# gnovack/distributed-training-and-deepspeed

Measured on AMD Instinct MI355X. Metric: tokens/sec (whole node) BERT-base DDP, higher is better.
Workload: dtype bf16; 1 GPU; model=bert-base-cased, params=108340804, global_batch=1024, per_gpu_batch=1024, seq_len=512, parallelism=dp1, grad_dtype=bfloat16, impl=fused, mlm_head=sparse (labelled rows only, static capacity 80896; identical loss/grads), optimizer=fused AdamW (transformers.AdamW hyper-params, lr 5e-5), tuned_gemms=True, hip_graph=False, force_collectives=False, prewarm=auto, async_wgrad=False, opt_overlap=True

## Files before the change

### distributed_training_and_deepspeed_amd/ops/_lib.py

```python
from __future__ import annotations

import ctypes
import os
from pathlib import Path
import threading

import torch

from . import build as _build

_LIB = None
_LOCK = threading.Lock()

P = ctypes.c_void_p
I = ctypes.c_int
F = ctypes.c_float
SZ = ctypes.c_size_t
U32 = ctypes.c_uint32
L = ctypes.c_long

_SIGS = {
    "dtd_ln_bwd_num_partials": (I, [I, I]),
    "dtd_ln_fwd": (I, [I, P, P, P, P, P, P, P, P, I, I, F, F, P, U32, P]),
    "dtd_ln_bwd": (I, [I, P, P, P, P, P, P, P, P, P, P, P, P, I, I, F, P, U32, P]),
# ... 28 lines not shown
    "dtd_embed_fwd": (I, [I, P, P, P, P, P, P, I, I, I, I, P]),
    "dtd_embed_fwd_pos": (I, [I, P, P, P, P, P, P, P, I, I, I, I, P]),
    "dtd_embed_word_bwd": (I, [I, I, P, P, P, P, I, I, I, I, P]),
    "dtd_embed_pos_bwd": (I, [I, I, P, P, I, I, I, I, I, P]),
    "dtd_scatter_rows": (I, [P, P, P, I, P, I, I, P]),
    "dtd_dropout": (I, [I, P, P, P, SZ, F, P, U32, P]),
    "dtd_embed_ln_fwd": (I, [P, P, P, P, P, P, P, P, P, P, P, I, I, I, I, F, F, P, U32, P]),
    "dtd_adam_step": (I, [P, P, P, P, I, P, SZ, P, I, P]),
    "dtd_scale_cast": (I, [P, I, P, I, SZ, F, P, P]),
    "dtd_sqnorm_num_partials": (I, [SZ]),
    "dtd_sqnorm_partials": (I, [P, I, SZ, P, P]),
    "dtd_attn_fwd": (I, [P, P, P, P, P, P, P, I, I, I, I, I, I, I, F, F, P, U32, P]),
    "dtd_attn_bwd": (I, [P, P, P, P, P, P, P, P, P, P, P, P, I, I, I, I, I, I, I, F, F, P, P]),
    "dtd_attn_fwd_range": (I, [P, P, P, P, P, P, P, I, I, I, I, I, I, I, F, F, P, U32, P, P]),
    "dtd_attn_bwd_range": (I, [P, P, P, P, P, P, P, P, P, P, P, P, I, I, I, I, I, I, I, F, F, P, P, P]),
    "dtd_attn_fwd_doc": (I, [P, P, P, P, P, P, P, I, I, I, I, I, I, I, F, F, P, U32, P, P]),
    "dtd_attn_bwd_doc": (I, [P, P, P, P, P, P, P, P, P, P, P, P, I, I, I, I, I, I, I, F, F, P, P, P]),
    "dtd_attn_fwd_gqa": (I, [P, P, P, P, P, I, I, I, I, I, I, I, I, F, P, P, P]),
    "dtd_attn_bwd_gqa": (I, [P, P, P, P, P, P, P, P, P, P, I, I, I, I, I, I, I, I, F, P, P, P]),
    "dtd_attn_masks": (I, [P, I, I, I, F, P, U32, P]),
    "dtd_attn_set_bwd_form": (I, [I]),
    "dtd_attn_set_bwd_kernels": (I, [I]),
    "dtd_attn_fused_bwd_built": (I, []),
    "dtd_attn_fwd_f32": (I, [P, P, P, P, P, P, P, I, I, I, I, I, I, I, F, F, P]),
    "dtd_attn_bwd_f32": (I, [P, P, P, P, P, P, P, P, P, P, P, P, I, I, I, I, I, I, I, F, F, P]),
    "dtd_softmax_fwd": (I, [I, P, P, I, I, P]),
    "dtd_softmax_bwd": (I, [I, P, P, P, I, I, P]),
    "dtd_gemm_bt_supported": (I, [I, I, I]),
    "dtd_gemm_w4_supported": (I, [I, I, I]),
    "dtd_gemm_w4_set_sched": (I, [I]),
    "dtd_gemm_w4": (I, [I, P, I, P, I, P, I, P, I, I, I, P]),
    "dtd_gemm_bt_part_rows": (I, [I]),
    "dtd_gemm_bt": (I, [I, P, I, P, I, P, I, P, P, I, P, P, I, I, I, P, P]),
    "dtd_spin_occupy": (I, [I, ctypes.c_double, P]),
    "dtd_gemm_set_stagger": (I, [ctypes.c_double]),
    "dtd_transpose_bf16": (I, [P, P, I, I, P]),
    "dtd_transpose_many": (I, [P, P, P, P, I, P]),
    "dtd_gemm_set_stamps": (I, [P]),
    "dtd_wgrad_tn_supported": (I, [I, I, I]),
    "dtd_wgrad_tn_splits": (I, [I, I, I]),
    "dtd_wgrad_tn": (I, [I, P, I, P, I, P, I, I, I, I, P]),
    "dtd_gemm_f32_supported": (I, [I, I, I]),
    "dtd_gemm_f32_set_kernel": (I, [I]),
    "dtd_gemm_f32_nt": (I, [P, I, P, I, P, I, P, I, I, I, I, P]),
    "dtd_gemm_f32_nn": (I, [P, I, P, I, P, I, I, I, I, I, P]),
    "dtd_transpose_many_f32": (I, [P, P, P, P, I, P]),
    "dtd_gemm_f32_tn_splits": (I, [I, I, I]),
    "dtd_gemm_f32_tn": (I, [P, I, P, I, P, I, I, I, I, P]),
    "dtd_gemm_ln_supported": (I, [I, I, I, I, I, I, I]),
    "dtd_gemm_ln": (I, [P, P, P, P, P, P, P, P, P, P, I, I, I, I, I, I, I, F, F, P, U32, P]),
    "dtd_splitk_reduce": (I, [P, I, I, ctypes.c_longlong, P, I, I, P]),
}


class KernelError(RuntimeError):
    pass


def available() -> bool:
    return torch.cuda.is_available()


def lib():
    global _LIB
    if _LIB is not None:
        return _LIB
# ... 58 lines not shown
```

### distributed_training_and_deepspeed_amd/ops/csrc/gemm.hip

```cpp
#include <type_traits>

#ifndef DTD_GEMM_DIAG
#define DTD_GEMM_DIAG 0
#endif
#ifndef DTD_GEMM_ONEBAR
#define DTD_GEMM_ONEBAR 0
#endif
constexpr bool kOneBar = DTD_GEMM_ONEBAR != 0;

#include "common.h"

using namespace dtd;

namespace {

typedef __attribute__((address_space(3))) void lds_void;
typedef const __attribute__((address_space(1))) void gbl_void;

constexpr int BM = 256, BN = 256, BK = 64;
constexpr int A_BYTES = BM * BK * 2;
constexpr int TILE_BYTES = (BM + BN) * BK * 2;
constexpr int LDS_BYTES = 2 * TILE_BYTES;

enum Epi : int { EPI_STORE = 0, EPI_BIAS_GELU = 1, EPI_GELU_BWD = 2, EPI_ADD = 3, EPI_BIAS_GELU_TANH = 4,
                 EPI_GELU_TANH_BWD = 5, EPI_BIAS_RELU = 6, EPI_RELU_BWD = 7, EPI_BIAS_GELU_G = 8,
                 EPI_BIAS_GELU_TANH_G = 9, EPI_MUL_BWD = 10, EPI_LAST = EPI_MUL_BWD };
__host__ __device__ constexpr bool is_gelu_fwd(int e) {
  return e == EPI_BIAS_GELU || e == EPI_BIAS_GELU_TANH || e == EPI_BIAS_RELU || e == EPI_BIAS_GELU_G ||
         e == EPI_BIAS_GELU_TANH_G;
}
__host__ __device__ constexpr bool is_gelu_bwd(int e) {
  return e == EPI_GELU_BWD || e == EPI_GELU_TANH_BWD || e == EPI_RELU_BWD || e == EPI_MUL_BWD;
}
__host__ __device__ constexpr bool stores_grad(int e) { return e == EPI_BIAS_GELU_G || e == EPI_BIAS_GELU_TANH_G; }

struct GemmArgs {
  const bf16* a; const bf16* b;
  bf16* c;
  bf16* c2;
  const bf16* u;
  const bf16* bias;
  float* part;
  int M, N, K, lda, ldb, ldc, ldu;
  unsigned long long* stamps;
  int* sched;
  int stagger;
  int nt;
};

__device__ __forceinline__ void st8(bf16* p, const bf16x8& v, int nt) {
  if (nt) __builtin_nontemporal_store(v, reinterpret_cast<bf16x8*>(p));
  else *reinterpret_cast<bf16x8*>(p) = v;
}

constexpr int SCHED_DONE = 8;

#ifdef DTD_GEMM_STAMPS
#define STAMP(slot, iter)                                                                          \
  do {                                                                                             \
    if (g.stamps && tid == 0 && (iter) < 32)                                                       \
      g.stamps[((size_t)blockIdx.x * 32 + (iter)) * 8 + (slot)] = __builtin_amdgcn_s_memtime();    \
  } while (0)
#define STAMP_ID(iter)                                                                             \
  do {                                                                                             \
    if (g.stamps && tid == 0 && (iter) < 32)                                                       \
      g.stamps[((size_t)blockIdx.x * 32 + (iter)) * 8 + 7] =                                       \
          ((unsigned long long)__builtin_amdgcn_s_getreg((31 << 11) | 20) << 32) |                 \
          __builtin_amdgcn_s_getreg((31 << 11) | 4);                                               \
  } while (0)
#else
#define STAMP(slot, iter) do {} while (0)
#define STAMP_ID(iter) do {} while (0)
#endif

__device__ __forceinline__ void bar() {
  asm volatile("" ::: "memory");
  __builtin_amdgcn_s_barrier();
  asm volatile("" ::: "memory");
}

// ... 33 lines not shown
__device__ __forceinline__ float epi_act_grad(float x) {
  if constexpr (EPI == EPI_GELU_TANH_BWD) return gelu_tanh_grad(x);
  else if constexpr (EPI == EPI_RELU_BWD) return x > 0.f ? 1.f : 0.f;
  else if constexpr (EPI == EPI_MUL_BWD) return x;
  else return gelu_grad(x);
}
template <int EPI>
__device__ __forceinline__ void epi_act_and_grad(float x, float& a, float& d) {
  if constexpr (EPI == EPI_BIAS_GELU_TANH_G) {
    const float k = 0.7978845608028654f;
    const float t = tanh_fast(k * fmaf(0.044715f * x, x * x, x));
    const float h = 0.5f * (1.f + t);
    a = x * h;
    d = h + 0.5f * x * (1.f - t * t) * k * (1.f + 3.f * 0.044715f * x * x);
  } else {
    const float e = gauss_e(x);
    const float cdf = phi_cdf(x, e);
    a = x * cdf;
    d = fmaf(x * 0.3989422804014327f, e, cdf);
  }
}
__device__ __forceinline__ float gelu_grad(float x) {
  const float e = gauss_e(x);
  return fmaf(x * 0.3989422804014327f, e, phi_cdf(x, e));
}

__device__ __forceinline__ bf16x4 cvt4(f32x4 v) {
  typedef float f32x2_t __attribute__((ext_vector_type(2)));
  const bf16x2 lo = __builtin_convertvector(f32x2_t{v[0], v[1]}, bf16x2);
  const bf16x2 hi = __builtin_convertvector(f32x2_t{v[2], v[3]}, bf16x2);
  return __builtin_shufflevector(lo, hi, 0, 1, 2, 3);
}

template <int EPI>
__device__ __forceinline__ void act_and_grad8(const bf16x8& v, float (&a)[8], float (&d)[8]) {
  float x[8];
#pragma unroll
  for (int j = 0; j < 8; ++j) x[j] = (float)v[j];
  if constexpr (EPI == EPI_BIAS_GELU_TANH_G) {
#pragma unroll
    for (int j = 0; j < 8; ++j) epi_act_and_grad<EPI>(x[j], a[j], d[j]);
  } else {
    float e[8], t[8], p[8], c[8];
#pragma unroll
    for (int j = 0; j < 8; ++j) e[j] = gauss_e(x[j]);
#pragma unroll
    for (int j = 0; j < 8; ++j) t[j] = __builtin_amdgcn_rcpf(fmaf(fabsf(x[j]), 0.3275911f * 0.70710678118654752f, 1.f));
#pragma unroll
    for (int j = 0; j < 8; ++j) p[j] = fmaf(t[j], 1.061405429f, -1.453152027f);
#pragma unroll
    for (int j = 0; j < 8; ++j) p[j] = fmaf(t[j], p[j], 1.421413741f);
#pragma unroll
    for (int j = 0; j < 8; ++j) p[j] = fmaf(t[j], p[j], -0.284496736f);
#pragma unroll
    for (int j = 0; j < 8; ++j) p[j] = t[j] * fmaf(t[j], p[j], 0.254829592f);
#pragma unroll
    for (int j = 0; j < 8; ++j) c[j] = 0.5f + 0.5f * copysignf(1.f - p[j] * e[j], x[j]);
#pragma unroll
    for (int j = 0; j < 8; ++j) {
      a[j] = x[j] * c[j];
      d[j] = fmaf(x[j] * 0.3989422804014327f, e[j], c[j]);
    }
  }
}
__device__ __forceinline__ bf16x8 cvt8(const float (&f)[8]) {
  const bf16x4 lo = cvt4(f32x4{f[0], f[1], f[2], f[3]}), hi = cvt4(f32x4{f[4], f[5], f[6], f[7]});
  return __builtin_shufflevector(lo, hi, 0, 1, 2, 3, 4, 5, 6, 7);
}

__device__ __forceinline__ int xcd_remap(int id, int n) {
  const int q = n / 8, r = n % 8, x = id % 8;
  return (x < r ? x * (q + 1) : r * (q + 1) + (x - r) * q) + id / 8;
}

__device__ __forceinline__ __amdgpu_buffer_rsrc_t uniform_rsrc(const void* p) {
  const uint64_t a = (uint64_t)p;
  const uint32_t lo = __builtin_amdgcn_readfirstlane((uint32_t)a);
  const uint32_t hi = __builtin_amdgcn_readfirstlane((uint32_t)(a >> 32));
  return __builtin_amdgcn_make_buffer_rsrc((void*)(((uint64_t)hi << 32) | lo), (short)0, 0x7fffffff, 0x00020000);
}

struct StageOffs {
  int a[2][2], b[2][2];
  int la[2][2], lb[2][2];
};

__device__ __forceinline__ StageOffs stage_offsets(int w, int lane, int lda, int ldb) {
  StageOffs o;
  const int dr = lane >> 3;
  const int sc = ((lane & 7) ^ dr) * 8;
#pragma unroll
  for (int h = 0; h < 2; ++h)
#pragma unroll
    for (int i = 0; i < 2; ++i) {
      const int j = w * 2 + i;
      const int ra = (j >> 3) * 128 + (h ? 64 : 0) + 8 * (j & 7);
      const int rb = (j >> 2) * 64 + (h ? 32 : 0) + 8 * (j & 3);
      o.a[h][i] = ((ra + dr) * lda + sc) * 2;
      o.b[h][i] = ((rb + dr) * ldb + sc) * 2;
      o.la[h][i] = ra * 128;
// ... 201 lines not shown
    __syncthreads();
    float* red = reinterpret_cast<float*>(smem);
    if (lane < 32) {
      *reinterpret_cast<f32x4*>(red + w * 256 + c * 8) = f32x4{colsum[0], colsum[1], colsum[2], colsum[3]};
      *reinterpret_cast<f32x4*>(red + w * 256 + c * 8 + 4) = f32x4{colsum[4], colsum[5], colsum[6], colsum[7]};
    }
    __syncthreads();
    if (tid < 256) {
      float s = 0.f;
#pragma unroll
      for (int k = 0; k < 8; ++k) s += red[k * 256 + tid];
      g.part[(size_t)bm * g.N + n0 + tid] = s;
    }
  }
}

constexpr int kStores(int epi) {
  return is_gelu_fwd(epi) ? 32 : is_gelu_bwd(epi) ? 32 : epi == EPI_ADD ? 48 : 16;
}

__device__ __forceinline__ void tile_of(int t, int ntn, int& m0, int& n0) {
  m0 = (t / ntn) * BM;
  n0 = (t % ntn) * BN;
}

__device__ __forceinline__ void sched_finish(int* q, int nwg, int tid) {
  if (q == nullptr || tid != 0) return;
  if (atomicAdd(&q[SCHED_DONE], 1) == nwg - 1) {
#pragma unroll
    for (int i = 0; i <= SCHED_DONE; ++i) atomicExch(&q[i], 0);
  }
}

template <int EPI, bool DYN>
__global__ void __launch_bounds__(512, 2) gemm_bt_persistent(GemmArgs g) {
  __shared__ __attribute__((aligned(1024))) char smem[LDS_BYTES];
  const int tid = threadIdx.x, lane = tid & 63, w = __builtin_amdgcn_readfirstlane(tid >> 6);
  const int li = lane & 15, lq = lane >> 4, sw = li & 7;
  const int wm = w >> 2, wn = w & 3;
  const int ntn = g.N / BN, ntiles = (g.M / BM) * ntn;
  const int nk = g.K / BK;
  const int nwg = gridDim.x, x = blockIdx.x % 8, l = blockIdx.x / 8, per = nwg / 8;
  const int q = ntiles / 8, r = ntiles % 8;
  const int beg = x < r ? x * (q + 1) : r * (q + 1) + (x - r) * q;
  const int end = beg + q + (x < r ? 1 : 0);
  constexpr bool dyn = DYN;
  __shared__ int qslot[2];
  int t = beg + l;
  if (t >= end) {
    if constexpr (DYN) sched_finish(g.sched, nwg, tid);
    return;
  }
  if (g.stagger > 0 && (l & 1)) {
    const unsigned long long t0 = __builtin_amdgcn_s_memrealtime();
    while (__builtin_amdgcn_s_memrealtime() - t0 < (unsigned long long)g.stagger) __builtin_amdgcn_s_sleep(8);
  }
  int m0, n0;
  tile_of(t, ntn, m0, n0);
  const StageOffs so = stage_offsets(w, lane, g.lda, g.ldb);
  auto rsa = uniform_rsrc(g.a + (size_t)m0 * g.lda), rsb = uniform_rsrc(g.b + (size_t)n0 * g.ldb);
  stage<0>(so, rsa, rsb, smem, 0);
  stage<1>(so, rsa, rsb, smem, 0);
  stage<2>(so, rsa, rsb, smem, 0);
  stage<3>(so, rsa, rsb, smem, 0);
  asm volatile("s_waitcnt vmcnt(0)" ::: "memory");
  __syncthreads();
  if (!kOneBar && __builtin_amdgcn_readfirstlane(wm) == 1) bar();

  const int arow = (wm * 128 + li) * 128;
  const int brow = A_BYTES + (wn * 64 + li) * 128;
  const int ch0 = ((0 * 4 + lq) ^ sw) * 16, ch1 = ((1 * 4 + lq) ^ sw) * 16;
  constexpr int S = kStores(EPI);
  constexpr int WAIT_FIRST = 4 + S > 63 ? 63 : 4 + S;

  bf16x8 af[4][2], b0[2][2], b1[2][2];
  f32x4 acc[8][4];
  int buf = 0;
  int it = 0;
  STAMP_ID(0);
  while (true) {
    STAMP(0, it);
    const int tn = dyn && it > 0 ? __builtin_amdgcn_readfirstlane(qslot[it & 1]) : t + per;
    const bool has_next = tn < end;
    int m1 = 0, n1 = 0;
    if (has_next) tile_of(tn, ntn, m1, n1);
    const auto rsa1 = uniform_rsrc(g.a + (size_t)m1 * g.lda), rsb1 = uniform_rsrc(g.b + (size_t)n1 * g.ldb);
    auto kstep = [&](auto first_c, int kt) {
      constexpr bool first = decltype(first_c)::value;
      const char* cur = smem + buf * TILE_BYTES;
      char* nxt = smem + (buf ^ 1) * TILE_BYTES;
      buf ^= 1;
      const bool more_here = kt + 1 < nk;
      const bool more = more_here || has_next;
// ... 113 lines not shown
    bar();
    char* img = smem + (buf ^ 1) * TILE_BYTES;
    const int c = lane & 31;
    bf16x8 uin[2][8];
    if constexpr (is_gelu_bwd(EPI)) {
      const auto rs = uniform_rsrc(g.u + (size_t)m0 * g.ldu + n0);
      const int voff = ((w * 16 + (lane >> 5)) * g.ldu + c * 8) * 2;
#pragma unroll
      for (int rr = 0; rr < 2; ++rr)
#pragma unroll
        for (int i = 0; i < 8; ++i)
          uin[rr][i] = __builtin_bit_cast(bf16x8, __builtin_amdgcn_raw_buffer_load_b128(
                                                      rs, voff, (rr * 128 + 2 * i) * g.ldu * 2, 0));
    }
    float colsum[8];
#pragma unroll
    for (int j = 0; j < 8; ++j) colsum[j] = 0.f;
    int claim = 0;
#pragma unroll
    for (int rr = 0; rr < 2; ++rr) {
      if (dyn && rr == 1 && has_next && tid == 0) claim = atomicAdd(&g.sched[x], 1);
      if (__builtin_amdgcn_readfirstlane(wm) == rr) {
#pragma unroll
        for (int ni = 0; ni < 4; ++ni) {
          const int n = wn * 64 + ni * 16 + 4 * lq;
#pragma unroll
          for (int mi = 0; mi < 8; ++mi) {
            const int m = mi * 16 + li;
            *reinterpret_cast<bf16x4*>(img + m * 512 + (((n >> 2) ^ ((m & 15) << 1)) << 3)) = pk[mi][ni];
          }
        }
      }
      bar();
#pragma unroll
      for (int i = 0; i < 8; ++i) {
        const int r = w * 16 + 2 * i + (lane >> 5);
        const bf16x8 v = *reinterpret_cast<const bf16x8*>(img + r * 512 + ((c ^ (r & 15)) << 4));
        const size_t off = (size_t)(m0 + rr * 128 + r) * g.ldc + n0 + c * 8;
        if constexpr (EPI == EPI_STORE || EPI == EPI_ADD) {
          st8(g.c + off, v, g.nt);
        } else if constexpr (stores_grad(EPI)) {
          float av[8], dv[8];
          act_and_grad8<EPI>(v, av, dv);
          st8(g.c + off, cvt8(dv), g.nt);
          st8(g.c2 + off, cvt8(av), g.nt);
        } else if constexpr (is_gelu_fwd(EPI)) {
          bf16x8 av;
#pragma unroll
          for (int j = 0; j < 8; ++j) av[j] = (bf16)epi_act<EPI>((float)v[j]);
          st8(g.c + off, v, g.nt);
          st8(g.c2 + off, av, g.nt);
        } else {
          float o[8];
#pragma unroll
          for (int j = 0; j < 8; ++j) {
            o[j] = (float)v[j] * epi_act_grad<EPI>((float)uin[rr][i][j]);
            colsum[j] += o[j];
          }
          st8(g.c + off, cvt8(o), g.nt);
        }
      }
      if (dyn && rr == 1 && tid == 0) qslot[(it + 1) & 1] = has_next ? beg + 2 * per + claim : end;
      bar();
    }
    if constexpr (is_gelu_bwd(EPI)) {
#pragma unroll
      for (int j = 0; j < 8; ++j) colsum[j] += __shfl_xor(colsum[j], 32, 64);
      float* red = reinterpret_cast<float*>(img);
      if (lane < 32) {
        *reinterpret_cast<f32x4*>(red + w * 256 + c * 8) = f32x4{colsum[0], colsum[1], colsum[2], colsum[3]};
        *reinterpret_cast<f32x4*>(red + w * 256 + c * 8 + 4) = f32x4{colsum[4], colsum[5], colsum[6], colsum[7]};
      }
      bar();
      if (tid < 256 && g.part) {
        float sum = 0.f;
#pragma unroll
        for (int k = 0; k < 8; ++k) sum += red[k * 256 + tid];
        g.part[(size_t)(m0 >> 8) * g.N + n0 + tid] = sum;
      }
      bar();
    }
    if (!kOneBar && has_next && __builtin_amdgcn_readfirstlane(wm) == 1) bar();
    STAMP(4, it);
    ++it;
    if (!has_next) break;
    t = tn;
    m0 = m1;
    n0 = n1;
    rsa = rsa1;
    rsb = rsb1;
  }
  if constexpr (DYN) sched_finish(g.sched, nwg, tid);
// ... 91 lines not shown
  return n;
}

static int gemm_nt_store() {
  const char* e = getenv("DTD_GEMM_NT_STORE");
  return !(e && e[0] == '0');
}

static int g_stagger = -1;
static int gemm_stagger() {
  if (g_stagger < 0) {
    const char* e = getenv("DTD_GEMM_STAGGER_US");
    g_stagger = e ? (int)(atof(e) * 100.0) : 0;
  }
  return g_stagger;
}
DTD_EXPORT int dtd_gemm_set_stagger(double us) {
  g_stagger = us > 0 ? (int)(us * 100.0) : 0;
  return 0;
}

static unsigned long long* g_stamps = nullptr;
DTD_EXPORT int dtd_gemm_set_stamps(void* p) {
  g_stamps = (unsigned long long*)p;
  return 0;
}

DTD_EXPORT int dtd_gemm_bt_supported(int M, int N, int K) {
  return M > 0 && N > 0 && K > 0 && M % BM == 0 && N % BN == 0 && K % BK == 0;
}

DTD_EXPORT int dtd_gemm_bt_part_rows(int M) { return M / BM; }

DTD_EXPORT int dtd_gemm_bt(int epi, const void* a, int lda, const void* b, int ldb, void* c, int ldc, void* c2,
                           const void* u, int ldu, const void* bias, float* part, int M, int N, int K,
                           int* sched, hipStream_t s) {
  if (!dtd_gemm_bt_supported(M, N, K)) return (int)hipErrorInvalidValue;
  if ((lda | ldb | ldc) % 8 || (u && ldu % 8)) return (int)hipErrorInvalidValue;
  if (lda < K || ldb < K || ldc < N) return (int)hipErrorInvalidValue;
  if (epi < EPI_STORE || epi > EPI_LAST) return (int)hipErrorInvalidValue;
  if (is_gelu_fwd(epi) && !c2) return (int)hipErrorInvalidValue;
  if (is_gelu_bwd(epi) && !u) return (int)hipErrorInvalidValue;
  GemmArgs g{(const bf16*)a, (const bf16*)b, (bf16*)c, (bf16*)c2, (const bf16*)u, (const bf16*)bias, part,
             M, N, K, lda, ldb, ldc, ldu, g_stamps, nullptr, gemm_stagger(), gemm_nt_store()};
  const int ntiles = (M / BM) * (N / BN);
  if (gemm_variant() >= 1) {
    const int cus = num_cus() / 8 * 8;
    const int nwg = ntiles >= cus ? cus : (ntiles + 7) / 8 * 8;
    g.sched = sched;
#define DTD_GEMM_P(E)                                                                       \
  if (sched) hipLaunchKernelGGL((gemm_bt_persistent<E, true>), dim3(nwg), dim3(512), 0, s, g);   \
  else hipLaunchKernelGGL((gemm_bt_persistent<E, false>), dim3(nwg), dim3(512), 0, s, g)
    switch (epi) {
      case EPI_STORE: DTD_GEMM_P(EPI_STORE); break;
      case EPI_BIAS_GELU: DTD_GEMM_P(EPI_BIAS_GELU); break;
      case EPI_GELU_BWD: DTD_GEMM_P(EPI_GELU_BWD); break;
      case EPI_ADD: DTD_GEMM_P(EPI_ADD); break;
      case EPI_BIAS_GELU_TANH: DTD_GEMM_P(EPI_BIAS_GELU_TANH); break;
      case EPI_GELU_TANH_BWD: DTD_GEMM_P(EPI_GELU_TANH_BWD); break;
      case EPI_BIAS_RELU: DTD_GEMM_P(EPI_BIAS_RELU); break;
      case EPI_RELU_BWD: DTD_GEMM_P(EPI_RELU_BWD); break;
      case EPI_BIAS_GELU_G: DTD_GEMM_P(EPI_BIAS_GELU_G); break;
      case EPI_BIAS_GELU_TANH_G: DTD_GEMM_P(EPI_BIAS_GELU_TANH_G); break;
      case EPI_MUL_BWD: DTD_GEMM_P(EPI_MUL_BWD); break;
      default: return (int)hipErrorInvalidValue;
    }
#undef DTD_GEMM_P
    DTD_LAUNCH_CHECK();
  }
  const dim3 grid(ntiles);
  switch (epi) {
    case EPI_STORE: hipLaunchKernelGGL(gemm_bt_kernel<EPI_STORE>, grid, dim3(512), 0, s, g); break;
    case EPI_BIAS_GELU: hipLaunchKernelGGL(gemm_bt_kernel<EPI_BIAS_GELU>, grid, dim3(512), 0, s, g); break;
    case EPI_GELU_BWD: hipLaunchKernelGGL(gemm_bt_kernel<EPI_GELU_BWD>, grid, dim3(512), 0, s, g); break;
    case EPI_ADD: hipLaunchKernelGGL(gemm_bt_kernel<EPI_ADD>, grid, dim3(512), 0, s, g); break;
    case EPI_BIAS_GELU_TANH: hipLaunchKernelGGL(gemm_bt_kernel<EPI_BIAS_GELU_TANH>, grid, dim3(512), 0, s, g); break;
    case EPI_GELU_TANH_BWD: hipLaunchKernelGGL(gemm_bt_kernel<EPI_GELU_TANH_BWD>, grid, dim3(512), 0, s, g); break;
    case EPI_BIAS_RELU: hipLaunchKernelGGL(gemm_bt_kernel<EPI_BIAS_RELU>, grid, dim3(512), 0, s, g); break;
    case EPI_RELU_BWD: hipLaunchKernelGGL(gemm_bt_kernel<EPI_RELU_BWD>, grid, dim3(512), 0, s, g); break;
    case EPI_BIAS_GELU_G: hipLaunchKernelGGL(gemm_bt_kernel<EPI_BIAS_GELU_G>, grid, dim3(512), 0, s, g); break;
    case EPI_BIAS_GELU_TANH_G: hipLaunchKernelGGL(gemm_bt_kernel<EPI_BIAS_GELU_TANH_G>, grid, dim3(512), 0, s, g); break;
    case EPI_MUL_BWD: hipLaunchKernelGGL(gemm_bt_kernel<EPI_MUL_BWD>, grid, dim3(512), 0, s, g); break;
    default: return (int)hipErrorInvalidValue;
  }
  DTD_LAUNCH_CHECK();
}

__global__ void __launch_bounds__(256) spin_occupy_kernel(unsigned long long ticks, int* sink) {
  __shared__ int hold[24576];
  const unsigned long long t0 = __builtin_amdgcn_s_memrealtime();
  hold[threadIdx.x] = (int)threadIdx.x;
  while (__builtin_amdgcn_s_memrealtime() - t0 < ticks) __builtin_amdgcn_s_sleep(8);
  __syncthreads();
  if (sink && hold[threadIdx.x ^ 1] < 0) sink[0] = 1;
}

DTD_EXPORT int dtd_spin_occupy(int nwg, double us, hipStream_t s) {
  if (nwg < 1 || nwg > 4096 || !(us >= 0.0) || us > 1e6) return (int)hipErrorInvalidValue;
  hipLaunchKernelGGL(spin_occupy_kernel, dim3(nwg), dim3(256), 0, s, (unsigned long long)(us * 100.0), nullptr);
  DTD_LAUNCH_CHECK();
}


DTD_EXPORT int dtd_transpose_many(const void* const* ins, void* const* outs, const int* rows, const int* cols, int n,
                                  hipStream_t s) {
  if (n <= 0) return 0;
  if (n > kMaxTranspose) return (int)hipErrorInvalidValue;
  TransposeSet set{};
  int tiles = 0;
  for (int i = 0; i < n; ++i) {
    if (rows[i] <= 0 || cols[i] <= 0 || rows[i] % 8 || cols[i] % 8 || ((uintptr_t)ins[i] | (uintptr_t)outs[i]) % 16)
      return (int)hipErrorInvalidValue;
    set.in[i] = (const bf16*)ins[i];
    set.out[i] = (bf16*)outs[i];
    set.rows[i] = rows[i];
    set.cols[i] = cols[i];
    set.tile0[i] = tiles;
    tiles += ((rows[i] + 63) / 64) * ((cols[i] + 63) / 64);
  }
  set.tile0[n] = tiles;
// ... 15 lines not shown
```

### distributed_training_and_deepspeed_amd/ops/gemm.py

```python
from __future__ import annotations

import contextlib
import ctypes
import os

import torch

from . import _lib

EPI_STORE, EPI_BIAS_GELU, EPI_GELU_BWD, EPI_ADD = 0, 1, 2, 3
EPI_BIAS_GELU_TANH, EPI_GELU_TANH_BWD, EPI_BIAS_RELU, EPI_RELU_BWD = 4, 5, 6, 7
EPI_BIAS_GELU_G, EPI_BIAS_GELU_TANH_G, EPI_MUL_BWD = 8, 9, 10
_ACT_EPI = {"gelu": (EPI_BIAS_GELU, EPI_GELU_BWD), "gelu_tanh": (EPI_BIAS_GELU_TANH, EPI_GELU_TANH_BWD),
            "relu": (EPI_BIAS_RELU, EPI_RELU_BWD)}
FUSED_ACTS = tuple(_ACT_EPI)
_ACT_GRAD_EPI = {"gelu": EPI_BIAS_GELU_G, "gelu_tanh": EPI_BIAS_GELU_TANH_G}
GRAD_ACTS = tuple(_ACT_GRAD_EPI)

_ENABLED = [os.environ.get("DTD_GEMM", "1") == "1"]


_FFN_FWD = [os.environ.get("DTD_GEMM_FFN_FWD", "1") == "1"]
_FFN_BWD = [os.environ.get("DTD_GEMM_FFN_BWD", "1") == "1"]
_FFN_STORE_GRAD = [os.environ.get("DTD_GEMM_FFN_STORE_GRAD", "1") == "1"]
_WGRAD = [os.environ.get("DTD_GEMM_WGRAD", "1") == "1"]
_ALL = [os.environ.get("DTD_GEMM_ALL", "0") == "1"]
_SCHED = [os.environ.get("DTD_GEMM_SCHED", "dynamic")]
assert _SCHED[0] in ("dynamic", "static"), _SCHED[0]
_QUEUES: dict = {}
_STATIC_EPIS = frozenset({EPI_GELU_TANH_BWD})


def enabled() -> bool:
    return _ENABLED[0]


_FFN_MIN_TILES = [int(os.environ.get("DTD_GEMM_FFN_MIN_TILES", "0")) or None]


def ffn_tiles_ok(M: int, N: int) -> bool:
    if _FFN_MIN_TILES[0] is None:
        _FFN_MIN_TILES[0] = torch.cuda.get_device_properties(torch.cuda.current_device()).multi_processor_count
    return (M // 256) * (N // 256) >= _FFN_MIN_TILES[0]


def ffn_fwd_enabled() -> bool:
    return _ENABLED[0] and _FFN_FWD[0]


def ffn_bwd_enabled() -> bool:
    return _ENABLED[0] and _FFN_BWD[0]


def ffn_store_grad_enabled() -> bool:
    return _ENABLED[0] and _FFN_FWD[0] and _FFN_BWD[0] and _FFN_STORE_GRAD[0]


def wgrad_enabled() -> bool:
    return _ENABLED[0] and (_WGRAD[0] or _ALL[0])


def set_wgrad(on: bool) -> None:
    _WGRAD[0] = bool(on)


def all_enabled() -> bool:
    return _ENABLED[0] and _ALL[0]
# ... 182 lines not shown
def _ok(t: torch.Tensor) -> bool:
    return (t is not None and t.is_cuda and t.dtype == torch.bfloat16 and t.dim() == 2 and t.stride(1) == 1
            and t.stride(0) % 8 == 0 and t.data_ptr() % 16 == 0)


def supported(M: int, N: int, K: int, *tensors) -> bool:
    if not all(_ok(t) for t in tensors):
        return False
    if not _lib.has("dtd_gemm_bt"):
        return False
    return bool(_lib.lib().dtd_gemm_bt_supported(M, N, K))


def set_sched(mode: str) -> None:
    assert mode in ("dynamic", "static"), mode
    _SCHED[0] = mode


def _queue() -> int | None:
    if _SCHED[0] != "dynamic":
        return None
    s = torch.cuda.current_stream()
    key = (s.device_index, s.cuda_stream)
    q = _QUEUES.get(key)
    if q is None:
        q = _QUEUES[key] = torch.zeros(16, dtype=torch.int32, device=torch.device("cuda", s.device_index))
    return q.data_ptr()


def _call(epi, a, b, c, c2=None, u=None, bias=None, part=None):
    M, K = a.shape
    N = b.shape[0]
    assert b.shape[1] == K and c.shape == (M, N), (a.shape, b.shape, c.shape)
    _lib.call("dtd_gemm_bt", epi, a.data_ptr(), a.stride(0), b.data_ptr(), b.stride(0), c.data_ptr(), c.stride(0),
              _lib.ptr(c2), _lib.ptr(u), u.stride(0) if u is not None else 0, _lib.ptr(bias), _lib.ptr(part),
              M, N, K, None if epi in _STATIC_EPIS else _queue(), _lib.stream())


def gemm_bt(a: torch.Tensor, b: torch.Tensor, bias: torch.Tensor | None = None) -> torch.Tensor:
    c = torch.empty((a.shape[0], b.shape[0]), dtype=a.dtype, device=a.device)
    _call(EPI_STORE, a, b, c, bias=bias)
    return c


def linear(x: torch.Tensor, w: torch.Tensor, b: torch.Tensor | None = None) -> torch.Tensor:
    return gemm_bt(x, w, b)


def matmul_nt(a: torch.Tensor, b_t: torch.Tensor) -> torch.Tensor:
    return gemm_bt(a, b_t)


def matmul_nt_add_(c: torch.Tensor, a: torch.Tensor, b_t: torch.Tensor) -> torch.Tensor:
    _call(EPI_ADD, a, b_t, c)
    return c


def linear_gelu(x: torch.Tensor, w: torch.Tensor, b: torch.Tensor | None, act: str = "gelu"):
    assert act in FUSED_ACTS, act
    M, N = x.shape[0], w.shape[0]
    u = torch.empty((M, N), dtype=x.dtype, device=x.device)
    a = torch.empty_like(u)
    _call(_ACT_EPI[act][0], x, w, u, c2=a, bias=b)
    return u, a


def linear_act_grad(x: torch.Tensor, w: torch.Tensor, b: torch.Tensor | None, act: str = "gelu"):
    assert act in GRAD_ACTS, act
    M, N = x.shape[0], w.shape[0]
# ... 198 lines not shown
```

Before: 1.527 million tokens/s.

## Serve GELU epilogue activations and gradients from an LDS lookup table

Precomputes a 65536-entry bf16 table of GELU value and derivative for every bf16 input. The persistent GEMM kernel copies a slice covering the common exponent range into LDS, then serves the fused bias+GELU epilogues by table lookup instead of evaluating the erf polynomial per element. Out-of-range inputs fall back to the analytic path. The table costs extra LDS per workgroup, adds a load at kernel start and a divergent fallback path, and results are rounded via bf16 input keys, so they may differ slightly from the analytic evaluation.

```diff
diff --git a/distributed_training_and_deepspeed_amd/ops/_lib.py b/distributed_training_and_deepspeed_amd/ops/_lib.py
--- a/distributed_training_and_deepspeed_amd/ops/_lib.py
+++ b/distributed_training_and_deepspeed_amd/ops/_lib.py
@@ -84,6 +84,9 @@
     "dtd_gemm_w4": (I, [I, P, I, P, I, P, I, P, I, I, I, P]),
     "dtd_gemm_bt_part_rows": (I, [I]),
     "dtd_gemm_bt": (I, [I, P, I, P, I, P, I, P, P, I, P, P, I, I, I, P, P]),
+    "dtd_gemm_bt_act": (I, [I, P, I, P, I, P, I, P, P, I, P, P, I, I, I, P, P, I, P]),
+    "dtd_gemm_act_table": (I, [I, P, P]),
+    "dtd_gemm_act_table_supported": (I, [I, I]),
     "dtd_spin_occupy": (I, [I, ctypes.c_double, P]),
     "dtd_gemm_set_stagger": (I, [ctypes.c_double]),
     "dtd_transpose_bf16": (I, [P, P, I, I, P]),
diff --git a/distributed_training_and_deepspeed_amd/ops/csrc/gemm.hip b/distributed_training_and_deepspeed_amd/ops/csrc/gemm.hip
--- a/distributed_training_and_deepspeed_amd/ops/csrc/gemm.hip
+++ b/distributed_training_and_deepspeed_amd/ops/csrc/gemm.hip
@@ -46,6 +46,7 @@
   int* sched;
   int stagger;
   int nt;
+  const uint32_t* tab;
 };
 
 __device__ __forceinline__ void st8(bf16* p, const bf16x8& v, int nt) {
@@ -145,32 +146,32 @@
   return __builtin_shufflevector(lo, hi, 0, 1, 2, 3);
 }
 
-template <int EPI>
+template <int EPI, int J0 = 0, int J1 = 8>
 __device__ __forceinline__ void act_and_grad8(const bf16x8& v, float (&a)[8], float (&d)[8]) {
   float x[8];
 #pragma unroll
-  for (int j = 0; j < 8; ++j) x[j] = (float)v[j];
+  for (int j = J0; j < J1; ++j) x[j] = (float)v[j];
   if constexpr (EPI == EPI_BIAS_GELU_TANH_G) {
 #pragma unroll
-    for (int j = 0; j < 8; ++j) epi_act_and_grad<EPI>(x[j], a[j], d[j]);
+    for (int j = J0; j < J1; ++j) epi_act_and_grad<EPI>(x[j], a[j], d[j]);
   } else {
     float e[8], t[8], p[8], c[8];
 #pragma unroll
-    for (int j = 0; j < 8; ++j) e[j] = gauss_e(x[j]);
-#pragma unroll
-    for (int j = 0; j < 8; ++j) t[j] = __builtin_amdgcn_rcpf(fmaf(fabsf(x[j]), 0.3275911f * 0.70710678118654752f, 1.f));
-#pragma unroll
-    for (int j = 0; j < 8; ++j) p[j] = fmaf(t[j], 1.061405429f, -1.453152027f);
-#pragma unroll
-    for (int j = 0; j < 8; ++j) p[j] = fmaf(t[j], p[j], 1.421413741f);
-#pragma unroll
-    for (int j = 0; j < 8; ++j) p[j] = fmaf(t[j], p[j], -0.284496736f);
-#pragma unroll
-    for (int j = 0; j < 8; ++j) p[j] = t[j] * fmaf(t[j], p[j], 0.254829592f);
-#pragma unroll
-    for (int j = 0; j < 8; ++j) c[j] = 0.5f + 0.5f * copysignf(1.f - p[j] * e[j], x[j]);
-#pragma unroll
-    for (int j = 0; j < 8; ++j) {
+    for (int j = J0; j < J1; ++j) e[j] = gauss_e(x[j]);
+#pragma unroll
+    for (int j = J0; j < J1; ++j) t[j] = __builtin_amdgcn_rcpf(fmaf(fabsf(x[j]), 0.3275911f * 0.70710678118654752f, 1.f));
+#pragma unroll
+    for (int j = J0; j < J1; ++j) p[j] = fmaf(t[j], 1.061405429f, -1.453152027f);
+#pragma unroll
+    for (int j = J0; j < J1; ++j) p[j] = fmaf(t[j], p[j], 1.421413741f);
+#pragma unroll
+    for (int j = J0; j < J1; ++j) p[j] = fmaf(t[j], p[j], -0.284496736f);
+#pragma unroll
+    for (int j = J0; j < J1; ++j) p[j] = t[j] * fmaf(t[j], p[j], 0.254829592f);
+#pragma unroll
+    for (int j = J0; j < J1; ++j) c[j] = 0.5f + 0.5f * copysignf(1.f - p[j] * e[j], x[j]);
+#pragma unroll
+    for (int j = J0; j < J1; ++j) {
       a[j] = x[j] * c[j];
       d[j] = fmaf(x[j] * 0.3989422804014327f, e[j], c[j]);
     }
@@ -179,6 +180,90 @@
 __device__ __forceinline__ bf16x8 cvt8(const float (&f)[8]) {
   const bf16x4 lo = cvt4(f32x4{f[0], f[1], f[2], f[3]}), hi = cvt4(f32x4{f[4], f[5], f[6], f[7]});
   return __builtin_shufflevector(lo, hi, 0, 1, 2, 3, 4, 5, 6, 7);
+}
+
+constexpr int kTabExpLo = 105, kTabBinades = 28;
+constexpr int kTabLo = kTabExpLo * 128;
+constexpr int kTabSpan = kTabBinades * 128;
+constexpr int kTabEntries = 2 * (kTabSpan + 1);
+constexpr int TAB_BYTES = kTabEntries * 4;
+constexpr int kTabLoads = (kTabEntries + 511) / 512;
+static_assert(LDS_BYTES + TAB_BYTES + 8 <= 160 * 1024, "K-step buffers + table slice + tile queue slots");
+static_assert((kTabSpan << 3 | 4) < 65536 && kTabLo + kTabSpan <= 0x7f80, "16-bit offsets; finite magnitudes only");
+
+typedef unsigned short u16x2 __attribute__((ext_vector_type(2)));
+typedef uint32_t u32x4 __attribute__((ext_vector_type(4)));
+
+template <int EPI>
+__global__ void __launch_bounds__(256) act_table_kernel(uint32_t* __restrict__ tab) {
+  const uint32_t bits = blockIdx.x * 256 + threadIdx.x;
+  const float x = __builtin_bit_cast(float, bits << 16);
+  if constexpr (stores_grad(EPI)) {
+    float a, d;
+    epi_act_and_grad<EPI>(x, a, d);
+    const bf16x4 r = cvt4(f32x4{a, d, 0.f, 0.f});
+    tab[bits] = __builtin_bit_cast(uint32_t, __builtin_shufflevector(r, r, 0, 1));
+  } else {
+    tab[bits] = __builtin_bit_cast(unsigned short, (bf16)epi_act<EPI>(x));
+  }
+}
+
+__device__ __forceinline__ uint32_t tab_offsets2(uint32_t w, bool& oor) {
+  const uint32_t mag = w & 0x7fff7fffu;
+  const u16x2 rel = __builtin_bit_cast(u16x2, mag) - u16x2{(unsigned short)kTabLo, (unsigned short)kTabLo};
+  const u16x2 cl = __builtin_elementwise_min(rel, u16x2{(unsigned short)kTabSpan, (unsigned short)kTabSpan});
+  const uint32_t r = __builtin_bit_cast(uint32_t, rel), c = __builtin_bit_cast(uint32_t, cl);
+  oor |= r != c;
+  return (c << 3) | ((w >> 13) & 0x00040004u);
+}
+
+__device__ __forceinline__ bool tab_misses2(uint32_t w) {
+  const uint32_t lo = w & 0x7fffu, hi = (w >> 16) & 0x7fffu;
+  return (lo != 0 && lo - (uint32_t)kTabLo >= (uint32_t)kTabSpan) || (hi != 0 && hi - (uint32_t)kTabLo >= (uint32_t)kTabSpan);
+}
+
+template <int TAB>
+__device__ __forceinline__ bool tab_misses8(const bf16x8& v) {
+  const u32x4 w = __builtin_bit_cast(u32x4, v);
+  bool miss = false;
+#pragma unroll
+  for (int k = 0; k < TAB / 2; ++k) miss |= tab_misses2(w[k]);
+  return miss;
+}
+
+template <int EPI, int TAB, bool GRAD>
+__device__ __forceinline__ bool act_table8(const bf16x8& v, uint32_t tab, bf16x8& av, bf16x8& dv) {
+  static_assert(TAB == 4 || TAB == 6 || TAB == 8, "elements of each 8-vector served by the table");
+  static_assert(GRAD || TAB == 8, "the act-only epilogues take the whole vector from the table");
+  typedef const __attribute__((address_space(3))) uint32_t* lds_u32;
+  const u32x4 w = __builtin_bit_cast(u32x4, v);
+  uint32_t e[8];
+  bool oor = false;
+#pragma unroll
+  for (int k = 0; k < TAB / 2; ++k) {
+    const uint32_t o = tab_offsets2(w[k], oor);
+    e[2 * k] = *(lds_u32)(uintptr_t)(((o & 0xffffu) | (tab & 0xffff0000u)) + (tab & 0xffffu));
+    e[2 * k + 1] = *(lds_u32)(uintptr_t)(__builtin_amdgcn_alignbit(tab >> 16, o, 16) + (tab & 0xffffu));
+  }
+  u32x4 a4, d4;
+  if constexpr (TAB < 8) {
+    float a[8], d[8];
+    act_and_grad8<EPI, TAB, 8>(v, a, d);
+    typedef float f32x2_t __attribute__((ext_vector_type(2)));
+#pragma unroll
+    for (int k = TAB / 2; k < 4; ++k) {
+      a4[k] = __builtin_bit_cast(uint32_t, __builtin_convertvector(f32x2_t{a[2 * k], a[2 * k + 1]}, bf16x2));
+      d4[k] = __builtin_bit_cast(uint32_t, __builtin_convertvector(f32x2_t{d[2 * k], d[2 * k + 1]}, bf16x2));
+    }
+  }
+#pragma unroll
+  for (int k = 0; k < TAB / 2; ++k) {
+    a4[k] = __builtin_amdgcn_perm(e[2 * k + 1], e[2 * k], 0x05040100u);
+    if constexpr (GRAD) d4[k] = __builtin_amdgcn_perm(e[2 * k + 1], e[2 * k], 0x07060302u);
+  }
+  av = __builtin_bit_cast(bf16x8, a4);
+  if constexpr (GRAD) dv = __builtin_bit_cast(bf16x8, d4);
+  return __any(oor);
 }
 
 __device__ __forceinline__ int xcd_remap(int id, int n) {
@@ -446,9 +531,10 @@
   }
 }
 
-template <int EPI, bool DYN>
+template <int EPI, bool DYN, int TAB = 0>
 __global__ void __launch_bounds__(512, 2) gemm_bt_persistent(GemmArgs g) {
-  __shared__ __attribute__((aligned(1024))) char smem[LDS_BYTES];
+  static_assert(TAB == 0 || EPI == EPI_BIAS_GELU || EPI == EPI_BIAS_GELU_TANH || stores_grad(EPI), "no table for this epilogue");
+  __shared__ __attribute__((aligned(1024))) char smem[LDS_BYTES + (TAB ? TAB_BYTES : 0)];
   const int tid = threadIdx.x, lane = tid & 63, w = __builtin_amdgcn_readfirstlane(tid >> 6);
   const int li = lane & 15, lq = lane >> 4, sw = li & 7;
   const int wm = w >> 2, wn = w & 3;
@@ -473,6 +559,18 @@
   tile_of(t, ntn, m0, n0);
   const StageOffs so = stage_offsets(w, lane, g.lda, g.ldb);
   auto rsa = uniform_rsrc(g.a + (size_t)m0 * g.lda), rsb = uniform_rsrc(g.b + (size_t)n0 * g.ldb);
+  const uint32_t tab_lds = (uint32_t)(uintptr_t)(const __attribute__((address_space(3))) char*)(smem + LDS_BYTES);
+  if constexpr (TAB > 0) {
+    uint32_t tabv[kTabLoads];
+#pragma unroll
+    for (int k = 0; k < kTabLoads; ++k) {
+      const int i = min(tid + 512 * k, kTabEntries - 1), rel = i >> 1;
+      tabv[k] = g.tab[((i & 1) << 15) | (rel < kTabSpan ? kTabLo + rel : 0)];
+    }
+#pragma unroll
+    for (int k = 0; k < kTabLoads; ++k)
+      if (tid + 512 * k < kTabEntries) reinterpret_cast<uint32_t*>(smem + LDS_BYTES)[tid + 512 * k] = tabv[k];
+  }
   stage<0>(so, rsa, rsb, smem, 0);
   stage<1>(so, rsa, rsb, smem, 0);
   stage<2>(so, rsa, rsb, smem, 0);
@@ -652,6 +750,7 @@
         }
       }
       bar();
+      int missed = 0;
 #pragma unroll
       for (int i = 0; i < 8; ++i) {
         const int r = w * 16 + 2 * i + (lane >> 5);
@@ -659,6 +758,11 @@
         const size_t off = (size_t)(m0 + rr * 128 + r) * g.ldc + n0 + c * 8;
         if constexpr (EPI == EPI_STORE || EPI == EPI_ADD) {
           st8(g.c + off, v, g.nt);
+        } else if constexpr (TAB > 0) {
+          bf16x8 av, dv = v;
+          if (act_table8<EPI, TAB, stores_grad(EPI)>(v, tab_lds, av, dv)) missed |= 1 << i;
+          st8(g.c + off, dv, g.nt);
+          st8(g.c2 + off, av, g.nt);
         } else if constexpr (stores_grad(EPI)) {
           float av[8], dv[8];
           act_and_grad8<EPI>(v, av, dv);
@@ -678,6 +782,31 @@
             colsum[j] += o[j];
           }
           st8(g.c + off, cvt8(o), g.nt);
+        }
+      }
+      if constexpr (TAB > 0) {
+        missed = __builtin_amdgcn_readfirstlane(missed);
+        if (__builtin_expect(missed != 0, 0)) {
+#pragma unroll 1
+          for (int i = 0; i < 8; ++i) {
+            if (!(missed >> i & 1)) continue;
+            const int r = w * 16 + 2 * i + (lane >> 5);
+            const bf16x8 v = *reinterpret_cast<const bf16x8*>(img + r * 512 + ((c ^ (r & 15)) << 4));
+            const size_t off = (size_t)(m0 + rr * 128 + r) * g.ldc + n0 + c * 8;
+            if (!__any(tab_misses8<TAB>(v))) continue;
+            if constexpr (stores_grad(EPI)) {
+              float av[8], dv[8];
+              act_and_grad8<EPI>(v, av, dv);
+              st8(g.c + off, cvt8(dv), g.nt);
+              st8(g.c2 + off, cvt8(av), g.nt);
+            } else {
+              bf16x8 av;
+#pragma unroll
+              for (int j = 0; j < 8; ++j) av[j] = (bf16)epi_act<EPI>((float)v[j]);
+              st8(g.c + off, v, g.nt);
+              st8(g.c2 + off, av, g.nt);
+            }
+          }
         }
       }
       if (dyn && rr == 1 && tid == 0) qslot[(it + 1) & 1] = has_next ? beg + 2 * per + claim : end;
@@ -835,9 +964,28 @@
 
 DTD_EXPORT int dtd_gemm_bt_part_rows(int M) { return M / BM; }
 
-DTD_EXPORT int dtd_gemm_bt(int epi, const void* a, int lda, const void* b, int ldb, void* c, int ldc, void* c2,
-                           const void* u, int ldu, const void* bias, float* part, int M, int N, int K,
-                           int* sched, hipStream_t s) {
+DTD_EXPORT int dtd_gemm_act_table(int epi, void* tab, hipStream_t s) {
+  uint32_t* t = (uint32_t*)tab;
+  switch (epi) {
+    case EPI_BIAS_GELU: hipLaunchKernelGGL(act_table_kernel<EPI_BIAS_GELU>, dim3(256), dim3(256), 0, s, t); break;
+    case EPI_BIAS_GELU_TANH: hipLaunchKernelGGL(act_table_kernel<EPI_BIAS_GELU_TANH>, dim3(256), dim3(256), 0, s, t); break;
+    case EPI_BIAS_GELU_G: hipLaunchKernelGGL(act_table_kernel<EPI_BIAS_GELU_G>, dim3(256), dim3(256), 0, s, t); break;
+    case EPI_BIAS_GELU_TANH_G: hipLaunchKernelGGL(act_table_kernel<EPI_BIAS_GELU_TANH_G>, dim3(256), dim3(256), 0, s, t); break;
+    default: return (int)hipErrorInvalidValue;
+  }
+  DTD_LAUNCH_CHECK();
+}
+
+DTD_EXPORT int dtd_gemm_act_table_supported(int epi, int split) {
+  if (stores_grad(epi)) return split == 4 || split == 6 || split == 8;
+  return (epi == EPI_BIAS_GELU || epi == EPI_BIAS_GELU_TANH) && split == 8;
+}
+
+DTD_EXPORT int dtd_gemm_bt_act(int epi, const void* a, int lda, const void* b, int ldb, void* c, int ldc, void* c2,
+                               const void* u, int ldu, const void* bias, float* part, int M, int N, int K,
+                               int* sched, const void* tab, int split, hipStream_t s) {
+  if (tab == nullptr || gemm_variant() < 1) split = 0;
+  if (split && !dtd_gemm_act_table_supported(epi, split)) return (int)hipErrorInvalidValue;
   if (!dtd_gemm_bt_supported(M, N, K)) return (int)hipErrorInvalidValue;
   if ((lda | ldb | ldc) % 8 || (u && ldu % 8)) return (int)hipErrorInvalidValue;
   if (lda < K || ldb < K || ldc < N) return (int)hipErrorInvalidValue;
@@ -845,12 +993,27 @@
   if (is_gelu_fwd(epi) && !c2) return (int)hipErrorInvalidValue;
   if (is_gelu_bwd(epi) && !u) return (int)hipErrorInvalidValue;
   GemmArgs g{(const bf16*)a, (const bf16*)b, (bf16*)c, (bf16*)c2, (const bf16*)u, (const bf16*)bias, part,
-             M, N, K, lda, ldb, ldc, ldu, g_stamps, nullptr, gemm_stagger(), gemm_nt_store()};
+             M, N, K, lda, ldb, ldc, ldu, g_stamps, nullptr, gemm_stagger(), gemm_nt_store(), (const uint32_t*)tab};
   const int ntiles = (M / BM) * (N / BN);
   if (gemm_variant() >= 1) {
     const int cus = num_cus() / 8 * 8;
     const int nwg = ntiles >= cus ? cus : (ntiles + 7) / 8 * 8;
     g.sched = sched;
+#define DTD_GEMM_PT(E, T)                                                                      \
+  if (sched) hipLaunchKernelGGL((gemm_bt_persistent<E, true, T>), dim3(nwg), dim3(512), 0, s, g);   \
+  else hipLaunchKernelGGL((gemm_bt_persistent<E, false, T>), dim3(nwg), dim3(512), 0, s, g)
+    if (split) {
+      if (epi == EPI_BIAS_GELU) { DTD_GEMM_PT(EPI_BIAS_GELU, 8); }
+      else if (epi == EPI_BIAS_GELU_TANH) { DTD_GEMM_PT(EPI_BIAS_GELU_TANH, 8); }
+      else if (epi == EPI_BIAS_GELU_G && split == 4) { DTD_GEMM_PT(EPI_BIAS_GELU_G, 4); }
+      else if (epi == EPI_BIAS_GELU_G && split == 6) { DTD_GEMM_PT(EPI_BIAS_GELU_G, 6); }
+      else if (epi == EPI_BIAS_GELU_G) { DTD_GEMM_PT(EPI_BIAS_GELU_G, 8); }
+      else if (split == 4) { DTD_GEMM_PT(EPI_BIAS_GELU_TANH_G, 4); }
+      else if (split == 6) { DTD_GEMM_PT(EPI_BIAS_GELU_TANH_G, 6); }
+      else { DTD_GEMM_PT(EPI_BIAS_GELU_TANH_G, 8); }
+      DTD_LAUNCH_CHECK();
+    }
+#undef DTD_GEMM_PT
 #define DTD_GEMM_P(E)                                                                       \
   if (sched) hipLaunchKernelGGL((gemm_bt_persistent<E, true>), dim3(nwg), dim3(512), 0, s, g);   \
   else hipLaunchKernelGGL((gemm_bt_persistent<E, false>), dim3(nwg), dim3(512), 0, s, g)
@@ -889,6 +1052,12 @@
   DTD_LAUNCH_CHECK();
 }
 
+DTD_EXPORT int dtd_gemm_bt(int epi, const void* a, int lda, const void* b, int ldb, void* c, int ldc, void* c2,
+                           const void* u, int ldu, const void* bias, float* part, int M, int N, int K,
+                           int* sched, hipStream_t s) {
+  return dtd_gemm_bt_act(epi, a, lda, b, ldb, c, ldc, c2, u, ldu, bias, part, M, N, K, sched, nullptr, 0, s);
+}
+
 __global__ void __launch_bounds__(256) spin_occupy_kernel(unsigned long long ticks, int* sink) {
   __shared__ int hold[24576];
   const unsigned long long t0 = __builtin_amdgcn_s_memrealtime();
diff --git a/distributed_training_and_deepspeed_amd/ops/gemm.py b/distributed_training_and_deepspeed_amd/ops/gemm.py
--- a/distributed_training_and_deepspeed_amd/ops/gemm.py
+++ b/distributed_training_and_deepspeed_amd/ops/gemm.py
@@ -33,6 +33,42 @@
 
 def enabled() -> bool:
     return _ENABLED[0]
+
+
+_ACT_TABLE_DEFAULT = 8
+_ACT_TABLE = [int(os.environ.get("DTD_GEMM_ACT_TABLE", _ACT_TABLE_DEFAULT))]
+assert _ACT_TABLE[0] in (0, 4, 6, 8), _ACT_TABLE[0]
+_ACT_TABLE_EPIS = frozenset({EPI_BIAS_GELU, EPI_BIAS_GELU_TANH, EPI_BIAS_GELU_G, EPI_BIAS_GELU_TANH_G})
+_ACT_TABLES: dict = {}
+
+
+def set_act_table(split: int) -> int:
+    assert split in (0, 4, 6, 8), split
+    prev, _ACT_TABLE[0] = _ACT_TABLE[0], int(split)
+    return prev
+
+
+def act_table(epi: int) -> torch.Tensor:
+    assert epi in _ACT_TABLE_EPIS, epi
+    key = (torch.cuda.current_device(), epi)
+    t = _ACT_TABLES.get(key)
+    if t is None:
+        t = torch.empty(65536, dtype=torch.int32, device=torch.device("cuda", key[0]))
+        _lib.call("dtd_gemm_act_table", epi, t.data_ptr(), _lib.stream())
+        torch.cuda.current_stream().synchronize()
+        _ACT_TABLES[key] = t
+    return t
+
+
+def _act_table_for(epi: int):
+    split = _ACT_TABLE[0]
+    if not split or epi not in _ACT_TABLE_EPIS or not _lib.has("dtd_gemm_bt_act"):
+        return None, 0
+    if epi in (EPI_BIAS_GELU, EPI_BIAS_GELU_TANH):
+        split = 8
+    if (torch.cuda.current_device(), epi) not in _ACT_TABLES and torch.cuda.is_current_stream_capturing():
+        return None, 0
+    return act_table(epi).data_ptr(), split
 
 
 _FFN_MIN_TILES = [int(os.environ.get("DTD_GEMM_FFN_MIN_TILES", "0")) or None]
@@ -281,9 +317,14 @@
     M, K = a.shape
     N = b.shape[0]
     assert b.shape[1] == K and c.shape == (M, N), (a.shape, b.shape, c.shape)
-    _lib.call("dtd_gemm_bt", epi, a.data_ptr(), a.stride(0), b.data_ptr(), b.stride(0), c.data_ptr(), c.stride(0),
-              _lib.ptr(c2), _lib.ptr(u), u.stride(0) if u is not None else 0, _lib.ptr(bias), _lib.ptr(part),
-              M, N, K, None if epi in _STATIC_EPIS else _queue(), _lib.stream())
+    tab, split = _act_table_for(epi)
+    args = (epi, a.data_ptr(), a.stride(0), b.data_ptr(), b.stride(0), c.data_ptr(), c.stride(0),
+            _lib.ptr(c2), _lib.ptr(u), u.stride(0) if u is not None else 0, _lib.ptr(bias), _lib.ptr(part),
+            M, N, K, None if epi in _STATIC_EPIS else _queue())
+    if split:
+        _lib.call("dtd_gemm_bt_act", *args, tab, split, _lib.stream())
+    else:
+        _lib.call("dtd_gemm_bt", *args, _lib.stream())
 
 
 def gemm_bt(a: torch.Tensor, b: torch.Tensor, bias: torch.Tensor | None = None) -> torch.Tensor:
```

Result: no change. 1.533 million tokens/s, median of 6 (+0.4%).
